# 959AI994/Multi-Gate-VAE

Hardware: AMD Instinct MI355X
Metric: circuit-graphs/sec (train step), AIG-64k batch=64 per GPU (higher is better)
Workload: dtype f32 storage; dense products as bf16x3 split-precision MFMA, fp32 accumulate; 1 GPU; cfg2: DG_AE --type aig, 64 x 65536-node synthetic levelised DAGs per GPU (N=4194304, E=6558720, 120 levels), H=64, 4+4 rounds, layernorm, weights [1,4,4], negatives sampled; step includes the 7-scalar metrics copy (pinned, read one step behind); global_batch=64, parallelism=dp1

## Files before the change

include/mgvae_hip.h:

```cpp
#ifndef MGVAE_HIP_H
#define MGVAE_HIP_H
#include <stdint.h>
#ifdef __cplusplus
extern "C" {
#endif

#ifndef MGV_OK
#define MGV_OK 0
#define MGV_EINVAL (-1)
#define MGV_EUNSUPPORTED (-2)
#endif

int mgv_abi_version(void);

int mgv_struct_stage_fwd(int H, int64_t N, const float* h_in, const int32_t* nbr_ptr, const int32_t* nbr_idx,
                         const uint8_t* xcls, const float* xtab, int C, const float* Wc, const float* bc,
                         const float* Whh, const float* bhh, const float* ln_w, const float* ln_b, float ln_eps,
                         float* h_out, void* stream);
int mgv_struct_stage_bwd(int H, int64_t N, const float* h_in, const int32_t* nbr_ptr, const int32_t* nbr_idx,
                         const uint8_t* xcls, const float* xtab, int C, const float* Wc, const float* WcT,
                         const float* bc, const float* Whh, const float* WhhT, const float* bhh,
                         const float* ln_w, const float* ln_b, float ln_eps, const float* gy_direct,
                         const float* gy_agg, float* g_direct_out, float* g_agg_out, float* dWc, float* dbc,
                         float* dWhh, float* dbhh, float* dxtab, float* dln_w, float* dln_b, void* stream);
// ... 100 lines not shown
                          int skip_inactive_longer_than ,
                          int heavy_active_n, const int32_t* heavy_nodes, const int32_t* heavy_node_seg_ptr, const int32_t* heavy_seg_e0,
                          const int32_t* heavy_seg_e1, const int32_t* heavy_lvl_k_ptr_host, const int32_t* heavy_lvl_seg_ptr_host,
                          float* heavy_ws, int skip_active_longer_than,
                          const float* gh, const float* h_prev, float* d_gh, float* g_hprev, void* stream);

int mgv_attn_pool_fwd(int W, int64_t N, const int32_t* in_ptr, const int32_t* in_src, const float* x, const float* u,
                      float* zbar, float* mstat, float* inv, void* stream);
int mgv_attn_pool_bwd(int W, int64_t N, const int32_t* in_ptr, const int32_t* in_src, const float* x, const float* u,
                      const float* zbar, const float* mstat, const float* inv, const float* dzbar, float* dx, float* du,
                      void* stream);

int mgv_sweep_pull_heavy(int H, int K, const int32_t* nodes, const int32_t* node_seg_ptr, int S, const int32_t* seg_e0,
                         const int32_t* seg_e1, const int32_t* out_dst, const int32_t* out_slot, const uint8_t* gslot,
                         const float* alpha, const float* dsc, const float* dzb, const float* attn_u, float* partial_ws,
                         float* ghs, void* stream);

int mgv_edge_dot_fwd(int H, int64_t E, const float* s, const float* t, int ld, const int64_t* src,
                     const int64_t* dst, int sigmoid, float* out, void* stream);
int mgv_edge_dot_bwd(int H, int64_t E, const float* s, const float* t, int ld, const int64_t* src,
                     const int64_t* dst, int sigmoid, const float* gout, float* ds, float* dt, void* stream);
int mgv_pair_scores_fwd(int H, int64_t M, int64_t N, const float* s, int lds, const float* t, int ldt, int sigmoid, float* out,
                        int64_t ldo, void* stream);
int mgv_pair_scores_bwd(int H, int64_t M, int64_t N, const float* s, int lds, const float* t, int ldt, int sigmoid, const float* out,
                        int64_t ldo, const float* gout, int64_t ldg, float* ds, int ldds, float* dt, int lddt, void* stream);
int mgv_pair_scores_at(int H, int64_t E, const float* s, int lds, const float* t, int ldt, const int64_t* src, const int64_t* dst,
                       int sigmoid, float* out, void* stream);
int mgv_pair_topk(int H, int64_t N, const float* s, int lds, const float* t, int ldt, const int32_t* graph_ptr, int G, int k, int sigmoid,
                  float threshold, int skip_self, int32_t* idx, float* score, int32_t* n_above, void* stream);
int mgv_recon_loss_fwd(int H, const float* s, const float* t, int ld, const int64_t* pos_src, const int64_t* pos_dst,
                       int64_t Epos, const int64_t* neg_src, const int64_t* neg_dst, int64_t Eneg,
                       double* sums, uint64_t* counts, int32_t* pred_bin, double* workspace, int64_t workspace_doubles,
                       void* stream);
int mgv_recon_loss_bwd(int H, int64_t N, const float* s, const float* t, int ld, const int64_t* pos_src, const int64_t* pos_dst,
                       int64_t Epos, const int32_t* pos_out_ptr, const int32_t* pos_out_dst, const int32_t* pos_in_ptr,
                       const int32_t* pos_in_src, const int64_t* neg_src, const int64_t* neg_dst, int64_t Eneg,
                       const float* gscale, float* ds, float* dt, void* stream);
int mgv_recon_loss_bwd_csr(int H, int64_t N, const float* s, const float* t, int ld, const int32_t* pos_out_ptr,
                           const int32_t* pos_out_dst, const int32_t* pos_in_ptr, const int32_t* pos_in_src, int64_t Epos,
                           const int32_t* neg_out_ptr, const int32_t* neg_out_dst, const int32_t* neg_in_ptr,
                           const int32_t* neg_in_src, int64_t Eneg, const float* gscale, float* ds, float* dt,
                           int skip_pos_longer_than , void* stream);
int mgv_recon_heavy_lists(int H, const float* s, const float* t, int ld, int64_t Epos, const float* gscale, int K,
                          const int32_t* nodes, const int32_t* node_seg_ptr, int S, const int32_t* seg_node, const int32_t* seg_e0,
                          const int32_t* seg_e1, const int32_t* list, int which, float* partial_ws, float* out, void* stream);
int mgv_link_keys(int H, const float* s, const float* t, int ld, const int64_t* pos_src, const int64_t* pos_dst, int64_t P,
                  const int64_t* neg_src, const int64_t* neg_dst, int64_t Q, uint32_t* keys, float* scores, int32_t* status,
                  void* stream);
int mgv_link_rank_work_ints(int64_t n);
int mgv_link_rank(int64_t n, int64_t P, const uint32_t* sorted_keys, const int32_t* order, double* out, int32_t* work,
                  int64_t work_ints, void* stream);
int mgv_neg_sample(int64_t N, int64_t E, uint64_t seed, const int32_t* pos_out_ptr, const int32_t* pos_out_dst,
                   int64_t* neg_src, int64_t* neg_dst, int32_t* cnt_out, int32_t* cnt_in, int32_t* rank_out, int32_t* rank_in,
                   void* stream);
int mgv_neg_bucket(int64_t E, const int64_t* neg_src, const int64_t* neg_dst, const int32_t* out_ptr, const int32_t* in_ptr,
                   const int32_t* rank_out, const int32_t* rank_in, int64_t* srt_src, int64_t* srt_dst, int32_t* out_dst, int32_t* in_src,
                   void* stream);

int mgv_func_loss_fwd(int H, int64_t P, const float* hf, const int64_t* pair_a, const int64_t* pair_b,
                      const float* tt, float eps, float* dis, double* ws, double* workspace, int64_t workspace_doubles,
                      void* stream);
int mgv_func_loss_bwd_csr(int H, int64_t N, int64_t P, const float* hf, const int64_t* pair_a, const int64_t* pair_b, const float* tt_sim,
                          const float* dis, float eps, const double* workspace8, const float* grad_loss, const int32_t* a_ptr,
                          const int32_t* a_pair, const int32_t* b_ptr, const int32_t* b_pair, const float* add, float* dhf, void* stream);
int mgv_func_loss_bwd(int H, int64_t P, const float* hf, const int64_t* pair_a, const int64_t* pair_b,
                      const float* tt, const float* dis, float eps, const double* ws, const float* gscale,
                      float* dhf, void* stream);

int mgv_reparam_fwd(int64_t n, const float* mu, const float* logstd, const float* eps, uint64_t seed,
                    float* eps_out, float* z, double* klsum, void* stream);
int mgv_reparam_bwd(int64_t n, const float* mu, const float* logstd, const float* eps, const float* gz,
                    const float* gkl, float klcoef, float* dmu, float* dlogstd, void* stream);
int mgv_confusion(int64_t n, const int32_t* pred_bin, const int32_t* gt_bin, uint64_t* counts, void* stream);

int mgv_sum_workspace_doubles(void);
int mgv_colstats(int64_t N, int C, const float* Y, int ld, double* sums, double* workspace, int64_t workspace_doubles, void* stream);
int mgv_bn_act_fwd(int64_t N, int C, const float* Y, const float* mean, const float* invstd, const float* gamma,
                   const float* beta, float p_drop, uint64_t seed, float* A, void* stream);
int mgv_bn_act_bwd(int64_t N, int C, const float* Y, const float* mean, const float* invstd, const float* gamma,
                   const float* beta, float p_drop, uint64_t seed, const float* dA, float* dZ, double* sums, double* workspace,
                   int64_t workspace_doubles, void* stream);
int mgv_bn_bwd_apply(int64_t N, int C, const float* Y, const float* mean, const float* invstd, const float* gamma,
                     const float* dZ, const double* sums, int batch_stats, float* dY, void* stream);
int mgv_readout_head_fwd(int64_t N, int C, const float* A, const float* w, const float* b, int clamp01, float* prob, void* stream);
int mgv_readout_head_bwd(int64_t N, int C, const float* A, const float* w, const float* b, int clamp01, const float* dprob,
                         float* dA, float* dw, float* db, double* workspace, int64_t workspace_doubles, void* stream);
int mgv_readout_fused_pack_elems(void);
int mgv_readout_fused_grad_floats(void);
int mgv_readout_fused_ws_doubles(int64_t N);
int mgv_readout_fused_fwd(int64_t N, const float* hf, const void* wpack, const float* b1, const float* g1, const float* be1,
// ... 75 lines not shown
```

multi-gate-vae_amd/csrc/losses.hip:

```cpp
#include "mgv_common.h"
#include "mgv_slab.h"
#include "../../include/mgvae_hip.h"

namespace mgv {

__device__ __forceinline__ void atomic_add4(float* p, const float4& v) {
    atomicAdd(p + 0, v.x); atomicAdd(p + 1, v.y); atomicAdd(p + 2, v.z); atomicAdd(p + 3, v.w);
}

__device__ __forceinline__ double block_sum_d(double v, double* red) {
    const int tid = threadIdx.x;
    __syncthreads();
    red[tid] = v;
    __syncthreads();
    for (int s = kThreads / 2; s > 0; s >>= 1) {
        if (tid < s) red[tid] += red[tid + s];
        __syncthreads();
    }
    return red[0];
}

template <int H, bool BWD>
__global__ __launch_bounds__(kThreads) void k_edge_dot(int64_t E, const float* s, const float* t, int ld,
                                                       const int64_t* src, const int64_t* dst, int sigmoid,
// ... 179 lines not shown
        }
        st4(ds + u * ld + 4 * lr, gs);
        st4(dt + u * ld + 4 * lr, gt);
    }
}

template <int H>
__global__ __launch_bounds__(256) void k_recon_heavy_seg(int S, const int32_t* seg_node, const int32_t* seg_e0, const int32_t* seg_e1,
                                                         const int32_t* nodes, const float* s, const float* t, int ld, const int32_t* list,
                                                         int which, int64_t Ep, const float* gscale, float* partial) {
    constexpr int LPR = H / 4, G = 256 / LPR;
    __shared__ __attribute__((aligned(16))) float s_p[G][H];
    const int lr = threadIdx.x % LPR, grp = threadIdx.x / LPR;
    const float wp = -(*gscale) / (float)Ep;
    for (int sg = blockIdx.x; sg < S; sg += gridDim.x) {
        const int64_t u = nodes[seg_node[sg]];
        const float4 own = ld4((which ? t : s) + u * ld + 4 * lr);
        const float* other = which ? s : t;
        float4 acc = zero4();
        for (int e = seg_e0[sg] + grp; e < seg_e1[sg]; e += G) {
            const float4 v = ld4(other + (int64_t)list[e] * ld + 4 * lr);
            const float p = sigmoidf_(group_sum<LPR>(dot4(own, v)));
            acc = fma4(wp * p * (1.0f - p) / (p + 1e-15f), v, acc);
        }
        __syncthreads();
        st4(&s_p[grp][4 * lr], acc);
        __syncthreads();
        if (grp == 0) {
            float4 tot = zero4();
            for (int g = 0; g < G; ++g) tot = add4(tot, ld4(&s_p[g][4 * lr]));
            st4(partial + (int64_t)sg * H + 4 * lr, tot);
        }
    }
}

template <int H>
__global__ __launch_bounds__(kThreads) void k_recon_bwd_rows(int64_t E, const float* s, const float* t, int ld, const int64_t* src,
                                                             const int64_t* dst, int negative, float wscale, const float* gscale,
                                                             float* ds, float* dt) {
    constexpr int EPB = kThreads / H;
    const int l = threadIdx.x % H, slot = threadIdx.x / H;
    const float w = (*gscale) * wscale;
    for (int64_t e0 = (int64_t)blockIdx.x * EPB; e0 < E; e0 += (int64_t)gridDim.x * EPB) {
        const int64_t e = e0 + slot;
        const bool ok = e < E;
        int64_t u = 0, v = 0;
        float x = 0.f, y = 0.f;
        if (ok) { u = src[e]; v = dst[e]; x = s[u * ld + l]; y = t[v * ld + l]; }
        const float p = sigmoidf_(group_sum<H>(x * y));
        if (!ok) continue;
        const float dp = p * (1.0f - p);
        const float c = negative ? w * dp / ((1.0f - p) + 1e-15f) : -w * dp / (p + 1e-15f);
        atomicAdd(ds + u * ld + l, c * y);
        atomicAdd(dt + v * ld + l, c * x);
    }
}

template <int H>
__global__ __launch_bounds__(kThreads) void k_func_dist(int64_t P, const float* hf, const int64_t* pa, const int64_t* pb,
                                                        const float* tt, float eps, float* dis, double* slab) {
    constexpr int LPR = H / 4, PPB = kThreads / LPR;
    __shared__ double red[kThreads];
    const int lr = threadIdx.x % LPR, slot = threadIdx.x / LPR;
    double sd = 0, sd2 = 0, st = 0, st2 = 0;
    for (int64_t p0 = (int64_t)blockIdx.x * PPB; p0 < P; p0 += (int64_t)gridDim.x * PPB) {
        const int64_t p = p0 + slot;
// ... 194 lines not shown
}

extern "C" int mgv_edge_dot_bwd(int H, int64_t E, const float* s, const float* t, int ld, const int64_t* src,
                                const int64_t* dst, int sigmoid, const float* gout, float* ds, float* dt, void* stream) {
    MGV_CHECK_ARG(E >= 0 && s && t && gout && ds && dt && ld >= H && ld % 4 == 0);
    if (E == 0) return MGV_OK;
    MGV_CHECK_ARG(src && dst);
    hipStream_t st = static_cast<hipStream_t>(stream);
    MGV_DISPATCH_H(H, hipLaunchKernelGGL((mgv::k_edge_dot<HH, true>), dim3(mgv::items_grid(E, mgv::kThreads / (HH / 4))), dim3(mgv::kThreads), 0, st,
                                         E, s, t, ld, src, dst, sigmoid, nullptr, gout, ds, dt));
    MGV_LAUNCH_RET();
}

extern "C" int mgv_recon_loss_fwd(int H, const float* s, const float* t, int ld, const int64_t* pos_src, const int64_t* pos_dst,
                                  int64_t Epos, const int64_t* neg_src, const int64_t* neg_dst, int64_t Eneg,
                                  double* sums, uint64_t* counts, int32_t* pred_bin, double* workspace, int64_t workspace_doubles,
                                  void* stream) {
    MGV_CHECK_ARG(s && t && sums && counts && Epos >= 0 && Eneg >= 0 && ld >= H && ld % 4 == 0);
    MGV_CHECK_ARG((Epos == 0 || (pos_src && pos_dst)) && (Eneg == 0 || (neg_src && neg_dst)));
    if (Epos + Eneg == 0) return MGV_OK;
    mgv::ReconArgs a{};
    a.s = s; a.t = t; a.ld = ld; a.psrc = pos_src; a.pdst = pos_dst; a.Ep = Epos; a.nsrc = neg_src; a.ndst = neg_dst; a.En = Eneg;
    a.sums = sums; a.cnt = reinterpret_cast<unsigned long long*>(counts); a.pred_bin = pred_bin;
    hipStream_t st = static_cast<hipStream_t>(stream);
    int grid = 0;
    MGV_DISPATCH_H(H, grid = mgv::items_grid(Epos + Eneg, mgv::kThreads / (HH / 4)));
    MGV_CHECK_ARG(workspace && workspace_doubles >= 2 * (int64_t)grid);
    a.slab = workspace;
    MGV_DISPATCH_H(H, hipLaunchKernelGGL((mgv::k_recon<HH, false>), dim3(grid), dim3(mgv::kThreads), 0, st, a));
    mgv::launch_slab_sum<double, double>(workspace, grid, 2, 2, sums, st);
    MGV_LAUNCH_RET();
}

extern "C" int mgv_recon_loss_bwd(int H, int64_t N, const float* s, const float* t, int ld, const int64_t* pos_src, const int64_t* pos_dst,
                                  int64_t Epos, const int32_t* pos_out_ptr, const int32_t* pos_out_dst, const int32_t* pos_in_ptr,
                                  const int32_t* pos_in_src, const int64_t* neg_src, const int64_t* neg_dst, int64_t Eneg,
                                  const float* gscale, float* ds, float* dt, void* stream) {
    MGV_CHECK_ARG(s && t && gscale && ds && dt && Epos >= 0 && Eneg >= 0 && N >= 0 && ld >= H && ld % 4 == 0);
    MGV_CHECK_ARG((Epos == 0 || (pos_src && pos_dst)) && (Eneg == 0 || (neg_src && neg_dst)));
    const bool pull = pos_out_ptr != nullptr;
    MGV_CHECK_ARG(!pull || (pos_in_ptr && (Epos == 0 || (pos_out_dst && pos_in_src))));
    if (H != 16 && H != 32 && H != 64) return MGV_EUNSUPPORTED;
    hipStream_t st = static_cast<hipStream_t>(stream);
    if (Epos > 0 && pull) {
        MGV_DISPATCH_H(H, hipLaunchKernelGGL((mgv::k_recon_bwd_pull<HH>), dim3(mgv::items_grid(N, mgv::kThreads / (HH / 4))), dim3(mgv::kThreads), 0, st,
                                             N, s, t, ld, pos_out_ptr, pos_out_dst, pos_in_ptr, pos_in_src, Epos, gscale, ds, dt));
    }
    for (int neg = (Epos > 0 && pull) ? 1 : 0; neg < 2; ++neg) {
        const int64_t E = neg ? Eneg : Epos;
        if (E == 0) continue;
        const int64_t* es = neg ? neg_src : pos_src;
        const int64_t* ed = neg ? neg_dst : pos_dst;
        const float wsc = 1.0f / (float)E;
        switch (H) {
            case 16: hipLaunchKernelGGL((mgv::k_recon_bwd_rows<16>), dim3(mgv::items_grid(E, mgv::kThreads / 16)), dim3(mgv::kThreads), 0, st, E, s, t, ld, es, ed, neg, wsc, gscale, ds, dt); break;
            case 32: hipLaunchKernelGGL((mgv::k_recon_bwd_rows<32>), dim3(mgv::items_grid(E, mgv::kThreads / 32)), dim3(mgv::kThreads), 0, st, E, s, t, ld, es, ed, neg, wsc, gscale, ds, dt); break;
            case 64: hipLaunchKernelGGL((mgv::k_recon_bwd_rows<64>), dim3(mgv::items_grid(E, mgv::kThreads / 64)), dim3(mgv::kThreads), 0, st, E, s, t, ld, es, ed, neg, wsc, gscale, ds, dt); break;
            default: return MGV_EUNSUPPORTED;
        }
    }
    MGV_LAUNCH_RET();
}

extern "C" int mgv_recon_loss_bwd_csr(int H, int64_t N, const float* s, const float* t, int ld, const int32_t* pos_out_ptr,
                                      const int32_t* pos_out_dst, const int32_t* pos_in_ptr, const int32_t* pos_in_src, int64_t Epos,
                                      const int32_t* neg_out_ptr, const int32_t* neg_out_dst, const int32_t* neg_in_ptr,
// ... 98 lines not shown
```

multi-gate-vae_amd/csrc/neg_sample.hip:

```cpp
#include "mgv_common.h"
#include "../../include/mgvae_hip.h"

namespace mgv {

__device__ __forceinline__ uint64_t splitmix64(uint64_t x) {
    x += 0x9E3779B97F4A7C15ull;
    x = (x ^ (x >> 30)) * 0xBF58476D1CE4E5B9ull;
    x = (x ^ (x >> 27)) * 0x94D049BB133111EBull;
    return x ^ (x >> 31);
}

__global__ __launch_bounds__(kThreads) void k_neg_sample(int64_t N, int64_t E, uint64_t seed, const int32_t* out_ptr, const int32_t* out_dst,
                                                        int64_t* neg_src, int64_t* neg_dst, int32_t* cnt_out, int32_t* cnt_in,
                                                        int32_t* rank_out, int32_t* rank_in) {
    for (int64_t i = (int64_t)blockIdx.x * kThreads + threadIdx.x; i < E; i += (int64_t)gridDim.x * kThreads) {
        uint64_t ctr = seed ^ ((uint64_t)i * 0xD1342543DE82EF95ull);
        int s, d;
        for (int attempt = 0;; ++attempt) {
            const uint64_t r = splitmix64(ctr + attempt);
            s = (int)(((r >> 32) * (uint64_t)N) >> 32);
            d = (int)(((r & 0xFFFFFFFFull) * (uint64_t)N) >> 32);
            bool ok = s != d;
            if (ok)
                for (int e = out_ptr[s]; e < out_ptr[s + 1]; ++e)
                    if (out_dst[e] == d) { ok = false; break; }
            if (ok || attempt >= 64) break;
        }
        neg_src[i] = s; neg_dst[i] = d;
        rank_out[i] = atomicAdd(cnt_out + s, 1);
        rank_in[i] = atomicAdd(cnt_in + d, 1);
    }
}

__global__ __launch_bounds__(kThreads) void k_neg_bucket(int64_t E, const int64_t* neg_src, const int64_t* neg_dst, const int32_t* out_ptr,
                                                        const int32_t* in_ptr, const int32_t* rank_out, const int32_t* rank_in, int64_t* srt_src,
                                                        int64_t* srt_dst, int32_t* out_dst, int32_t* in_src) {
    for (int64_t i = (int64_t)blockIdx.x * kThreads + threadIdx.x; i < E; i += (int64_t)gridDim.x * kThreads) {
        const int s = (int)neg_src[i], d = (int)neg_dst[i];
        const int p = out_ptr[s] + rank_out[i];
        srt_src[p] = s; srt_dst[p] = d; out_dst[p] = d;
        in_src[in_ptr[d] + rank_in[i]] = s;
    }
}

}

extern "C" int mgv_neg_sample(int64_t N, int64_t E, uint64_t seed, const int32_t* pos_out_ptr, const int32_t* pos_out_dst,
                              int64_t* neg_src, int64_t* neg_dst, int32_t* cnt_out, int32_t* cnt_in, int32_t* rank_out, int32_t* rank_in,
                              void* stream) {
    MGV_CHECK_ARG(N >= 2 && N < (1ll << 31) && E >= 0 && pos_out_ptr && neg_src && neg_dst && cnt_out && cnt_in && rank_out && rank_in);
    if (E == 0) return MGV_OK;
    hipLaunchKernelGGL(mgv::k_neg_sample, dim3(mgv::grid_for((E + mgv::kThreads - 1) / mgv::kThreads, 16)), dim3(mgv::kThreads), 0,
                       static_cast<hipStream_t>(stream), N, E, seed, pos_out_ptr, pos_out_dst, neg_src, neg_dst, cnt_out, cnt_in, rank_out, rank_in);
    MGV_LAUNCH_RET();
}

extern "C" int mgv_neg_bucket(int64_t E, const int64_t* neg_src, const int64_t* neg_dst, const int32_t* out_ptr, const int32_t* in_ptr,
                              const int32_t* rank_out, const int32_t* rank_in, int64_t* srt_src, int64_t* srt_dst, int32_t* out_dst, int32_t* in_src,
                              void* stream) {
    MGV_CHECK_ARG(E >= 0 && out_ptr && in_ptr && rank_out && rank_in);
    if (E == 0) return MGV_OK;
    MGV_CHECK_ARG(neg_src && neg_dst && srt_src && srt_dst && out_dst && in_src);
    hipLaunchKernelGGL(mgv::k_neg_bucket, dim3(mgv::grid_for((E + mgv::kThreads - 1) / mgv::kThreads, 16)), dim3(mgv::kThreads), 0,
                       static_cast<hipStream_t>(stream), E, neg_src, neg_dst, out_ptr, in_ptr, rank_out, rank_in, srt_src, srt_dst, out_dst, in_src);
    MGV_LAUNCH_RET();
}
```

multi-gate-vae_amd/deepgate/_model_base.py:

```python
import os

import torch
from torch import nn

from . import ops
from .arch.mlp import MLP
from .arch.tfmlp import TFMlpAggr
from .data import plan_of
from .digae_layer import DirectedInnerProductDecoder
from .sampling import NegativeEdges, negative_sampling, negative_sampling_device

EPS = 1e-15
DEVICE_SAMPLER = True
MAX_LOGSTD = 10


class FunctionalModel(nn.Module):
    ENCODER_ATTR = 'struct_encoder'
    GATES = ()

    def __init__(self, struct_encoder, num_rounds=1, dim_hidden=128, enable_encode=True, enable_reverse=True):
        super().__init__()
        setattr(self, self.ENCODER_ATTR, struct_encoder)
        self.decoder = DirectedInnerProductDecoder()
# ... 73 lines not shown
    def _decoder_halves(self, hs):
        st = ops.linear(hs.detach(), self.hs_decompose.weight, self.hs_decompose.bias)
        H = st.shape[1] // 2
        return st[:, :H], st[:, H:]

    def predict_links(self, hs, k, graph_ptr=None, skip_self=True):
        with torch.no_grad():
            s, t = self._decoder_halves(hs)
            return ops.pair_topk(s, t, k, graph_ptr=graph_ptr, sigmoid=True, threshold=0.5, skip_self=skip_self)

    def reconstruction_counts(self, hs, edge_index, graph_ptr, threshold=0.5):
        with torch.no_grad():
            s, t = self._decoder_halves(hs)
            return ops.reconstruction_counts(s, t, edge_index, graph_ptr, threshold)

    def recon_loss(self, hs, pos_edge_index, neg_edge_index=None, want_pred=True, edge_keys=None, plan=None, pass_hs=False, want_rank=False):
        if pass_hs and hs.requires_grad:
            st, self._hs_pass = ops.linear_passthrough(hs, self.hs_decompose.weight, self.hs_decompose.bias)
        else:
            st = ops.linear(hs, self.hs_decompose.weight, self.hs_decompose.bias)
        if plan is not None and (plan.E != pos_edge_index.shape[1] or plan.N != hs.shape[0]):
            plan = None
        neg_csr = None
        if neg_edge_index is None:
            neg_edge_index = self._draw_negatives(hs, pos_edge_index, plan, edge_keys)
        if plan is not None and hs.is_cuda and torch.is_tensor(neg_edge_index) and neg_edge_index.shape[1] > 0:
            cache = getattr(plan, '_neg_cache', None)
            key = (neg_edge_index.data_ptr(), neg_edge_index._version, tuple(neg_edge_index.shape), hs.shape[0])
            if cache is None or cache[0] is not neg_edge_index or cache[1] != key:
                from .sampling import bucket_negatives
                cache = plan._neg_cache = (neg_edge_index, key, bucket_negatives(neg_edge_index.long(), hs.shape[0]))
            neg_edge_index = cache[2]
        if isinstance(neg_edge_index, NegativeEdges):
            neg_csr, neg_edge_index = neg_edge_index.csr, neg_edge_index.edge_index
        loss, counts, pred_bin = ops.ReconLossFn.apply(st, pos_edge_index, neg_edge_index, want_pred, plan, neg_csr)
        self.last_confusion = counts
        self.last_link_metrics = ops.link_record(st, None, pos_edge_index, neg_edge_index) if want_rank else None
        Ep, En = pos_edge_index.shape[1], neg_edge_index.shape[1]
        gt_bin = None
        if want_pred:
            gt_bin = torch.zeros(Ep + En, dtype=torch.int32, device=hs.device)
            gt_bin[:Ep] = 1
        return loss, pred_bin if want_pred else None, gt_bin

    def load(self, model_path):
        checkpoint = torch.load(model_path, map_location=lambda storage, loc: storage)
        src = checkpoint['state_dict']
        state = {}
        for k, v in src.items():
            state[k[7:] if k.startswith('module') and not k.startswith('module_list') else k] = v
        own = self.state_dict()
        for k in list(state):
            if k in own:
                if state[k].shape != own[k].shape:
                    print('Skip loading parameter {}, required shape{}, loaded shape{}.'.format(k, own[k].shape, state[k].shape))
                    state[k] = own[k]
            else:
                print('Drop parameter {}.'.format(k))
        for k in own:
            if k not in state:
                print('No param {}.'.format(k))
                state[k] = own[k]
        self.load_state_dict(state, strict=False)

    def load_pretrained(self, pretrained_model_path=''):
        if pretrained_model_path == '':
            pretrained_model_path = os.path.join(os.path.dirname(__file__), 'pretrained', 'model.pth')
        self.load(pretrained_model_path)
```

multi-gate-vae_amd/deepgate/ops.py:

```python
import torch

from . import _hip
from ._hip import HipLibraryError, check, ptr

import os

F32 = torch.float32
I32 = torch.int32
U8 = torch.uint8
LN_EPS = 1e-5

PRECISION = os.environ.get('MGV_PRECISION', 'x3')
FIRST_STAGE_TABLE = True


def use_x3(H):
    return PRECISION == 'x3' and H in (32, 64)


def split_bf16(w):
    hi = w.to(torch.bfloat16)
    lo = (w - hi.to(torch.float32)).to(torch.bfloat16)
    return hi, lo

# ... 913 lines not shown
              ptr(idx), ptr(score), ptr(n_above))
    return idx, score, n_above


def reconstruction_counts(s, t, edge_index, graph_ptr, threshold=0.5):
    dev = s.device
    gp = torch.as_tensor(graph_ptr).to(device=dev, dtype=torch.int64)
    G = gp.numel() - 1
    src, dst = _edge_rows(edge_index)
    _, _, n_above = pair_topk(s, t, 1, graph_ptr=gp, sigmoid=True, threshold=threshold, skip_self=False)
    if G <= 0:
        return torch.zeros((0, 4), dtype=torch.int64, device=dev)
    hit = (pair_scores_at(s, t, edge_index, sigmoid=True) > threshold).to(torch.int64)
    gid = torch.bucketize(src, gp[1:].contiguous(), right=True).clamp_(max=G - 1)
    tp = torch.zeros(G, dtype=torch.int64, device=dev).index_add_(0, gid, hit)
    edges = torch.zeros(G, dtype=torch.int64, device=dev).index_add_(0, gid, torch.ones_like(hit))
    cs = torch.zeros(s.shape[0] + 1, dtype=torch.int64, device=dev)
    cs[1:] = torch.cumsum(n_above.to(torch.int64), 0)
    n = gp[1:] - gp[:-1]
    return torch.stack([tp, cs[gp[1:]] - cs[gp[:-1]], edges, n * n], dim=1)


def dense_scores(s, t):
    return pair_scores(s, t, sigmoid=False)


class ReconLossFn(torch.autograd.Function):

    @staticmethod
    def forward(ctx, st, pos_edge_index, neg_edge_index, want_pred, plan=None, neg_csr=None):
        std = check(st.detach().contiguous(), F32, 'st')
        N, H2 = std.shape
        H = H2 // 2
        ps, pd = _edge_rows(pos_edge_index)
        ns, nd = _edge_rows(neg_edge_index)
        Ep, En = ps.numel(), ns.numel()
        dev = std.device
        sums = torch.zeros(2, dtype=torch.float64, device=dev)
        counts = torch.zeros(4, dtype=torch.int64, device=dev)
        pred = torch.empty(Ep + En, dtype=torch.int32, device=dev) if want_pred else None
        t_view = std[:, H:]
        _hip.call('mgv_recon_loss_fwd', H, ptr(std), ptr(t_view), H2, ptr(ps), ptr(pd), Ep, ptr(ns), ptr(nd), En,
                  ptr(sums), ptr(counts), ptr(pred), *_sw(std.device))
        loss = (sums[0] / max(Ep, 1) + sums[1] / max(En, 1)).to(F32)
        ctx.save_for_backward(std, ps, pd, ns, nd)
        ctx.plan, ctx.neg_csr = plan, neg_csr
        ctx.mark_non_differentiable(counts)
        if pred is not None:
            ctx.mark_non_differentiable(pred)
            return loss, counts, pred
        return loss, counts, torch.empty(0, dtype=torch.int32, device=dev)

    @staticmethod
    def backward(ctx, gloss, _gc, _gp):
        global _SWEEP_BWD_EVENT
        if _SWEEP_BWD_EVENT is not None and gloss.is_cuda:
            torch.cuda.current_stream().wait_event(_SWEEP_BWD_EVENT)
            _SWEEP_BWD_EVENT = None
        std, ps, pd, ns, nd = ctx.saved_tensors
        H2 = std.shape[1]
        H = H2 // 2
        g = gloss.detach().to(F32).reshape(1).contiguous()
        pl = ctx.plan
        if pl is not None and ctx.neg_csr is not None:
            dst_ = torch.empty_like(std)
            heavy = [(0, pl.heavy_segments(True), pl.out_dst), (1, pl.heavy_segments(False), pl.in_src)]
            skip = pl.HEAVY_ROW if any(hv is not None for _, hv, _ in heavy) else 0
            _hip.call('mgv_recon_loss_bwd_csr', H, std.shape[0], ptr(std), ptr(std[:, H:]), H2, ptr(pl.out_ptr), ptr(pl.out_dst),
                      ptr(pl.in_ptr), ptr(pl.in_src), ps.numel(), *[ptr(c) for c in ctx.neg_csr], ns.numel(), ptr(g), ptr(dst_),
                      ptr(dst_[:, H:]), skip)
            for which, hv, lst in heavy:
                if hv is not None:
                    pw = workspace(hv['S'] * H, std.device)
                    _hip.call('mgv_recon_heavy_lists', H, ptr(std), ptr(std[:, H:]), H2, ps.numel(), ptr(g), hv['K'], ptr(hv['nodes']),
                              ptr(hv['node_seg_ptr']), hv['S'], ptr(hv['seg_node']), ptr(hv['seg_e0']), ptr(hv['seg_e1']), ptr(lst), which,
                              ptr(pw), ptr(dst_[:, H:]) if which else ptr(dst_))
            return dst_, None, None, None, None, None
        dst_ = torch.zeros_like(std)
        csr = (pl.out_ptr, pl.out_dst, pl.in_ptr, pl.in_src) if pl is not None else (None, None, None, None)
        _hip.call('mgv_recon_loss_bwd', H, std.shape[0], ptr(std), ptr(std[:, H:]), H2, ptr(ps), ptr(pd), ps.numel(),
                  *[ptr(c) for c in csr], ptr(ns), ptr(nd), ns.numel(), ptr(g), ptr(dst_), ptr(dst_[:, H:]))
        return dst_, None, None, None, None, None


def confusion_counts(pred_bin, gt_bin):
    counts = torch.zeros(4, dtype=torch.int64, device=pred_bin.device)
    _hip.call('mgv_confusion', pred_bin.numel(), ptr(check(pred_bin.contiguous(), torch.int32, 'pred_bin')),
              ptr(check(gt_bin.contiguous(), torch.int32, 'gt_bin')), ptr(counts))
    return counts


LINK_RECORD_WORDS = 8


def link_record(st_or_s, t=None, pos_edge_index=None, neg_edge_index=None, return_scores=False):
    neg = getattr(neg_edge_index, 'edge_index', neg_edge_index)
    P, Q = int(pos_edge_index.shape[1]), int(neg.shape[1])
    if P == 0 or Q == 0:
        raise ValueError('Only one class present (%d positive, %d negative pairs): ROC-AUC and average precision are not defined' % (P, Q))
    sd = check(st_or_s.detach().contiguous(), F32, 'st' if t is None else 's')
    if t is None:
        ld = sd.shape[1]
        H = ld // 2
        td = sd[:, H:]
    else:
        td = check(t.detach().contiguous(), F32, 't')
        ld = H = sd.shape[1]
        if td.shape != sd.shape:
            raise HipLibraryError('s and t must have the same shape (got %s and %s)' % (tuple(sd.shape), tuple(td.shape)))
    n = P + Q
# ... 288 lines not shown
```

multi-gate-vae_amd/deepgate/sampling.py:

```python
import itertools

import torch

from . import _hip
from ._hip import ptr

_CALLS = itertools.count()


class NegativeEdges:

    def __init__(self, edge_index, out_ptr, out_dst, in_ptr, in_src):
        self.edge_index, self.out_ptr, self.out_dst, self.in_ptr, self.in_src = edge_index, out_ptr, out_dst, in_ptr, in_src

    @property
    def csr(self):
        return self.out_ptr, self.out_dst, self.in_ptr, self.in_src


def bucket_negatives(neg, N):
    dev = neg.device
    E = int(neg.shape[1])
    i32 = dict(dtype=torch.int32, device=dev)
    src, dst = neg[0].contiguous(), neg[1].contiguous()
    in_ptr, out_ptr = torch.empty(N + 1, **i32), torch.empty(N + 1, **i32)
    in_src, in_dst, out_dst, out_slot = (torch.empty(max(E, 1), **i32) for _ in range(4))
    n_s = _hip.call_value('mgv_plan_csr_scratch_ints', N, E)
    scratch = torch.empty(n_s, **i32)
    status = torch.empty(2, **i32)
    _hip.call('mgv_plan_csr', N, E, ptr(src), ptr(dst), ptr(in_ptr), ptr(in_src), ptr(in_dst), ptr(out_ptr), ptr(out_dst), ptr(out_slot),
              None, None, ptr(scratch), n_s, ptr(status))
    if int(status[0].item()) != 0:
        raise ValueError('neg_edge_index holds node ids outside [0, num_nodes)')
    counts = (out_ptr[1:] - out_ptr[:-1]).long()
    srt_src = torch.repeat_interleave(torch.arange(N, device=dev), counts, output_size=E)
    srt = torch.stack([srt_src, out_dst[:E].long()])
    return NegativeEdges(srt, out_ptr, out_dst, in_ptr, in_src)


def negative_sampling_device(plan, num_neg_samples=None, generator=None):
    N, dev = plan.N, plan.device
    if getattr(plan, 'num_self_loops', None) is None:
        plan.count_self_loops()
    E = (plan.E - plan.num_self_loops) + N if num_neg_samples is None else int(num_neg_samples)
    base = generator.initial_seed() if generator is not None else torch.initial_seed()
    seed = (base * 0x9E3779B97F4A7C15 + next(_CALLS) * 0xD1B54A32D192ED03 + 0x2545F4914F6CDD1D) & 0xFFFFFFFFFFFFFFFF
    scratch = torch.zeros(2, N, dtype=torch.int32, device=dev)
    neg = torch.empty(2, E, dtype=torch.int64, device=dev)
    rank = torch.empty(2, max(E, 1), dtype=torch.int32, device=dev)
    _hip.call('mgv_neg_sample', N, E, seed, ptr(plan.out_ptr), ptr(plan.out_dst), ptr(neg[0]), ptr(neg[1]), ptr(scratch[0]), ptr(scratch[1]),
              ptr(rank[0]), ptr(rank[1]))
    ptrs = torch.zeros(2, N + 1, dtype=torch.int32, device=dev)
    for k in range(2):
        ptrs[k, 1:] = torch.cumsum(scratch[k], 0, dtype=torch.int32)
    srt = torch.empty(2, E, dtype=torch.int64, device=dev)
    out_dst = torch.empty(max(E, 1), dtype=torch.int32, device=dev)
    in_src = torch.empty(max(E, 1), dtype=torch.int32, device=dev)
    _hip.call('mgv_neg_bucket', E, ptr(neg[0]), ptr(neg[1]), ptr(ptrs[0]), ptr(ptrs[1]), ptr(rank[0]), ptr(rank[1]),
              ptr(srt[0]), ptr(srt[1]), ptr(out_dst), ptr(in_src))
    ss = torch.empty(N + 1 + E, dtype=torch.int32, device=dev)
    _hip.call('mgv_sort_lists_i32', N, E, ptr(ptrs[0]), ptr(out_dst), ptr(ss), ss.numel())
    _hip.call('mgv_sort_lists_i32', N, E, ptr(ptrs[1]), ptr(in_src), ptr(ss), ss.numel())
    srt[1].copy_(out_dst[:E])
    return NegativeEdges(srt, ptrs[0], out_dst, ptrs[1], in_src)


def sorted_edge_keys(pos_edge_index, num_nodes):
    src, dst = pos_edge_index[0].long(), pos_edge_index[1].long()
    keep = src != dst
    return torch.sort(src[keep] * int(num_nodes) + dst[keep]).values


def negative_sampling(pos_edge_index, num_nodes, num_neg_samples=None, generator=None, keys=None):
    dev = pos_edge_index.device
    N = int(num_nodes)
    if keys is None:
        keys = sorted_edge_keys(pos_edge_index, N)
    want = int(keys.numel()) + N if num_neg_samples is None else int(num_neg_samples)
    out = torch.empty((2, 0), dtype=torch.long, device=dev)
    guard = 0
    while out.shape[1] < want:
        m = want - out.shape[1]
        m = m + m // 8 + 16
        s = torch.randint(0, N, (m,), device=dev, generator=generator)
        d = torch.randint(0, N, (m,), device=dev, generator=generator)
        k = s * N + d
        ok = s != d
        if keys.numel() > 0:
            pos = torch.searchsorted(keys, k).clamp_(max=keys.numel() - 1)
            ok &= keys[pos] != k
        out = torch.cat([out, torch.stack([s[ok], d[ok]])], dim=1)
        guard += 1
        if guard > 64:
            raise RuntimeError('negative_sampling: graph too dense to draw %d non-edges' % want)
    return out[:, :want].contiguous()
```

Before: 982.3 graphs/s.

## Compute recon loss forward from CSR lists and sample negatives as packed int32

```diff
diff --git a/include/mgvae_hip.h b/include/mgvae_hip.h
--- a/include/mgvae_hip.h
+++ b/include/mgvae_hip.h
@@ -156,6 +156,11 @@
                        int64_t Epos, const int64_t* neg_src, const int64_t* neg_dst, int64_t Eneg,
                        double* sums, uint64_t* counts, int32_t* pred_bin, double* workspace, int64_t workspace_doubles,
                        void* stream);
+int mgv_recon_loss_fwd_csr(int H, int64_t N, const float* s, const float* t, int ld, const int32_t* pos_out_ptr,
+                           const int32_t* pos_out_dst, int64_t Epos, const int32_t* neg_out_ptr, const int32_t* neg_out_dst,
+                           int64_t Eneg, int skip_pos_longer_than, const int32_t* heavy_nodes, int S, const int32_t* seg_node,
+                           const int32_t* seg_e0, const int32_t* seg_e1, double* sums, uint64_t* counts, double* workspace,
+                           int64_t workspace_doubles, void* stream);
 int mgv_recon_loss_bwd(int H, int64_t N, const float* s, const float* t, int ld, const int64_t* pos_src, const int64_t* pos_dst,
                        int64_t Epos, const int32_t* pos_out_ptr, const int32_t* pos_out_dst, const int32_t* pos_in_ptr,
                        const int32_t* pos_in_src, const int64_t* neg_src, const int64_t* neg_dst, int64_t Eneg,
@@ -180,6 +185,10 @@
 int mgv_neg_bucket(int64_t E, const int64_t* neg_src, const int64_t* neg_dst, const int32_t* out_ptr, const int32_t* in_ptr,
                    const int32_t* rank_out, const int32_t* rank_in, int64_t* srt_src, int64_t* srt_dst, int32_t* out_dst, int32_t* in_src,
                    void* stream);
+int mgv_neg_sample_i32(int64_t N, int64_t E, uint64_t seed, const int32_t* pos_out_ptr, const int32_t* pos_out_dst,
+                       int32_t* pair, int32_t* cnt_out, int32_t* cnt_in, int32_t* rank, void* stream);
+int mgv_neg_bucket_i32(int64_t E, const int32_t* pair, const int32_t* out_ptr, const int32_t* in_ptr, const int32_t* rank,
+                       int32_t* out_dst, int32_t* in_src, void* stream);
 
 int mgv_func_loss_fwd(int H, int64_t P, const float* hf, const int64_t* pair_a, const int64_t* pair_b,
                       const float* tt, float eps, float* dis, double* ws, double* workspace, int64_t workspace_doubles,
diff --git a/multi-gate-vae_amd/csrc/losses.hip b/multi-gate-vae_amd/csrc/losses.hip
--- a/multi-gate-vae_amd/csrc/losses.hip
+++ b/multi-gate-vae_amd/csrc/losses.hip
@@ -235,6 +235,111 @@
             st4(partial + (int64_t)sg * H + 4 * lr, tot);
         }
     }
+}
+
+__device__ __forceinline__ float dot4_pairwise_rounded(const float4& a, const float4& b) {
+#pragma clang fp contract(off)
+    const float p0 = a.x * b.x, p1 = a.y * b.y, p2 = a.z * b.z, p3 = a.w * b.w;
+    return ((p0 + p1) + p2) + p3;
+}
+
+struct ReconTally {
+    double lp = 0, ln = 0;
+    unsigned int tp = 0, fp = 0, tn = 0, fn = 0;
+    __device__ __forceinline__ void add(float p, bool pos) {
+        const bool hit = p > 0.5f;
+        if (pos) { lp += (double)(-logf(p + 1e-15f)); tp += hit; fn += !hit; }
+        else     { ln += (double)(-logf((1.0f - p) + 1e-15f)); fp += hit; tn += !hit; }
+    }
+    __device__ __forceinline__ void flush(double* red, double* row, unsigned long long* cnt) {
+        const double sp = block_sum_d(lp, red), sn = block_sum_d(ln, red);
+        const double c0 = block_sum_d((double)tp, red), c1 = block_sum_d((double)fp, red);
+        const double c2 = block_sum_d((double)tn, red), c3 = block_sum_d((double)fn, red);
+        if (threadIdx.x == 0) {
+            row[0] = sp; row[1] = sn;
+            if (c0 > 0) atomicAdd(cnt + 0, (unsigned long long)c0);
+            if (c1 > 0) atomicAdd(cnt + 1, (unsigned long long)c1);
+            if (c2 > 0) atomicAdd(cnt + 2, (unsigned long long)c2);
+            if (c3 > 0) atomicAdd(cnt + 3, (unsigned long long)c3);
+        }
+    }
+};
+
+template <int H>
+__global__ __launch_bounds__(kThreads) void k_recon_fwd_lists(int64_t N, const float* s, const float* t, int ld, const int32_t* pout_ptr,
+                                                              const int32_t* pout_dst, int64_t Ep, const int32_t* nout_ptr,
+                                                              const int32_t* nout_dst, int64_t En, int skip_len, double* slab,
+                                                              unsigned long long* cnt) {
+    constexpr int LPR = H / 4, RPB = kThreads / LPR, K = 4;
+    __shared__ double red[kThreads];
+    const int lr = threadIdx.x % LPR, slot = threadIdx.x / LPR;
+    int64_t first, end, stride;
+    if ((gridDim.x & 7) == 0) {
+        const int64_t chunk = ((N + 8 * RPB - 1) / (8 * RPB)) * RPB;
+        first = (blockIdx.x & 7) * chunk + (int64_t)(blockIdx.x >> 3) * RPB;
+        end = min(N, ((blockIdx.x & 7) + 1) * chunk);
+        stride = (int64_t)(gridDim.x >> 3) * RPB;
+    } else {
+        first = (int64_t)blockIdx.x * RPB; end = N; stride = (int64_t)gridDim.x * RPB;
+    }
+    ReconTally tally;
+    for (int64_t n0 = first; n0 < end; n0 += stride) {
+        const int64_t u = n0 + slot;
+        if (u >= end) continue;
+        int b0 = 0, b1 = 0, c0 = 0, c1 = 0;
+        if (Ep > 0) {
+            b0 = pout_ptr[u]; c0 = pout_ptr[u + 1] - b0;
+            if (skip_len > 0 && c0 > skip_len) c0 = 0;
+        }
+        if (En > 0) { b1 = nout_ptr[u]; c1 = nout_ptr[u + 1] - b1; }
+        c1 += c0;
+        if (c1 == 0) continue;
+        const float4 su = ld4(s + u * ld + 4 * lr);
+        auto partner = [&](int j) -> int { return j < c0 ? pout_dst[b0 + j] : nout_dst[b1 + (j - c0)]; };
+        int id[K];
+#pragma unroll
+        for (int k = 0; k < K; ++k) id[k] = k < c1 ? partner(k) : 0;
+        for (int j0 = 0; j0 < c1; j0 += K) {
+            float4 v[K];
+#pragma unroll
+            for (int k = 0; k < K; ++k)
+                if (j0 + k < c1) v[k] = ld4(t + (int64_t)id[k] * ld + 4 * lr);
+            int nid[K];
+#pragma unroll
+            for (int k = 0; k < K; ++k) nid[k] = j0 + K + k < c1 ? partner(j0 + K + k) : 0;
+#pragma unroll
+            for (int k = 0; k < K; ++k) {
+                const int j = j0 + k;
+                if (j < c1) {
+                    const float p = sigmoidf_(group_sum<LPR>(dot4_pairwise_rounded(su, v[k])));
+                    if (lr == 0) tally.add(p, j < c0);
+                }
+            }
+#pragma unroll
+            for (int k = 0; k < K; ++k) id[k] = nid[k];
+        }
+    }
+    tally.flush(red, slab + 2 * (int64_t)blockIdx.x, cnt);
+}
+
+template <int H>
+__global__ __launch_bounds__(kThreads) void k_recon_fwd_heavy_seg(int S, const int32_t* seg_node, const int32_t* seg_e0, const int32_t* seg_e1,
+                                                                  const int32_t* nodes, const float* s, const float* t, int ld,
+                                                                  const int32_t* list, double* slab, unsigned long long* cnt) {
+    constexpr int LPR = H / 4, G = kThreads / LPR;
+    __shared__ double red[kThreads];
+    const int lr = threadIdx.x % LPR, grp = threadIdx.x / LPR;
+    ReconTally tally;
+    for (int sg = blockIdx.x; sg < S; sg += gridDim.x) {
+        const int64_t u = nodes[seg_node[sg]];
+        const float4 su = ld4(s + u * ld + 4 * lr);
+        for (int e = seg_e0[sg] + grp; e < seg_e1[sg]; e += G) {
+            const float4 v = ld4(t + (int64_t)list[e] * ld + 4 * lr);
+            const float p = sigmoidf_(group_sum<LPR>(dot4_pairwise_rounded(su, v)));
+            if (lr == 0) tally.add(p, true);
+        }
+    }
+    tally.flush(red, slab + 2 * (int64_t)blockIdx.x, cnt);
 }
 
 template <int H>
@@ -495,6 +600,31 @@
     MGV_LAUNCH_RET();
 }
 
+extern "C" int mgv_recon_loss_fwd_csr(int H, int64_t N, const float* s, const float* t, int ld, const int32_t* pos_out_ptr,
+                                      const int32_t* pos_out_dst, int64_t Epos, const int32_t* neg_out_ptr, const int32_t* neg_out_dst,
+                                      int64_t Eneg, int skip_pos_longer_than, const int32_t* heavy_nodes, int S, const int32_t* seg_node,
+                                      const int32_t* seg_e0, const int32_t* seg_e1, double* sums, uint64_t* counts, double* workspace,
+                                      int64_t workspace_doubles, void* stream) {
+    MGV_CHECK_ARG(s && t && sums && counts && Epos >= 0 && Eneg >= 0 && N >= 0 && ld >= H && ld % 4 == 0 && skip_pos_longer_than >= 0 && S >= 0);
+    MGV_CHECK_ARG(Epos == 0 || (pos_out_ptr && pos_out_dst));
+    MGV_CHECK_ARG(Eneg == 0 || (neg_out_ptr && neg_out_dst));
+    MGV_CHECK_ARG((skip_pos_longer_than > 0) == (S > 0) && (S == 0 || (Epos > 0 && heavy_nodes && seg_node && seg_e0 && seg_e1)));
+    if (H != 16 && H != 32 && H != 64 && H != 128) return MGV_EUNSUPPORTED;
+    if (N == 0 || Epos + Eneg == 0) return MGV_OK;
+    const int grid = mgv::items_grid(N, mgv::kThreads / (H / 4)), hgrid = S < 2048 ? S : 2048;
+    MGV_CHECK_ARG(workspace && workspace_doubles >= 2 * (int64_t)(grid + hgrid));
+    hipStream_t st = static_cast<hipStream_t>(stream);
+    unsigned long long* cnt = reinterpret_cast<unsigned long long*>(counts);
+    MGV_DISPATCH_H(H, hipLaunchKernelGGL((mgv::k_recon_fwd_lists<HH>), dim3(grid), dim3(mgv::kThreads), 0, st, N, s, t, ld, pos_out_ptr, pos_out_dst,
+                                         Epos, neg_out_ptr, neg_out_dst, Eneg, skip_pos_longer_than, workspace, cnt));
+    if (S > 0) {
+        MGV_DISPATCH_H(H, hipLaunchKernelGGL((mgv::k_recon_fwd_heavy_seg<HH>), dim3(hgrid), dim3(mgv::kThreads), 0, st, S, seg_node, seg_e0, seg_e1,
+                                             heavy_nodes, s, t, ld, pos_out_dst, workspace + 2 * (int64_t)grid, cnt));
+    }
+    mgv::launch_slab_sum<double, double>(workspace, grid + hgrid, 2, 2, sums, st);
+    MGV_LAUNCH_RET();
+}
+
 extern "C" int mgv_recon_loss_bwd(int H, int64_t N, const float* s, const float* t, int ld, const int64_t* pos_src, const int64_t* pos_dst,
                                   int64_t Epos, const int32_t* pos_out_ptr, const int32_t* pos_out_dst, const int32_t* pos_in_ptr,
                                   const int32_t* pos_in_src, const int64_t* neg_src, const int64_t* neg_dst, int64_t Eneg,
diff --git a/multi-gate-vae_amd/csrc/neg_sample.hip b/multi-gate-vae_amd/csrc/neg_sample.hip
--- a/multi-gate-vae_amd/csrc/neg_sample.hip
+++ b/multi-gate-vae_amd/csrc/neg_sample.hip
@@ -43,6 +43,59 @@
     }
 }
 
+__global__ __launch_bounds__(kThreads) void k_neg_sample_i32(int64_t N, int64_t E, uint64_t seed, const int32_t* out_ptr, const int32_t* out_dst,
+                                                            int2* pair, int32_t* cnt_out, int32_t* cnt_in, int2* rank) {
+    for (int64_t i = (int64_t)blockIdx.x * kThreads + threadIdx.x; i < E; i += (int64_t)gridDim.x * kThreads) {
+        uint64_t ctr = seed ^ ((uint64_t)i * 0xD1342543DE82EF95ull);
+        int s, d;
+        for (int attempt = 0;; ++attempt) {
+            const uint64_t r = splitmix64(ctr + attempt);
+            s = (int)(((r >> 32) * (uint64_t)N) >> 32);
+            d = (int)(((r & 0xFFFFFFFFull) * (uint64_t)N) >> 32);
+            bool ok = s != d;
+            if (ok)
+                for (int e = out_ptr[s]; e < out_ptr[s + 1]; ++e)
+                    if (out_dst[e] == d) { ok = false; break; }
+            if (ok || attempt >= 64) break;
+        }
+        pair[i] = make_int2(s, d);
+        const int ro = atomicAdd(cnt_out + s, 1), ri = atomicAdd(cnt_in + d, 1);
+        rank[i] = make_int2(ro, ri);
+    }
+}
+
+__global__ __launch_bounds__(kThreads) void k_neg_bucket_i32(int64_t E, const int2* pair, const int32_t* out_ptr, const int32_t* in_ptr,
+                                                            const int2* rank, int32_t* out_dst, int32_t* in_src) {
+    for (int64_t i = (int64_t)blockIdx.x * kThreads + threadIdx.x; i < E; i += (int64_t)gridDim.x * kThreads) {
+        const int2 p = pair[i], r = rank[i];
+        out_dst[out_ptr[p.x] + r.x] = p.y;
+        in_src[in_ptr[p.y] + r.y] = p.x;
+    }
+}
+
+}
+
+extern "C" int mgv_neg_sample_i32(int64_t N, int64_t E, uint64_t seed, const int32_t* pos_out_ptr, const int32_t* pos_out_dst,
+                                  int32_t* pair, int32_t* cnt_out, int32_t* cnt_in, int32_t* rank, void* stream) {
+    MGV_CHECK_ARG(N >= 2 && N < (1ll << 31) && E >= 0 && E < (1ll << 31) && pos_out_ptr && pair && cnt_out && cnt_in && rank);
+    MGV_CHECK_ARG((reinterpret_cast<uintptr_t>(pair) & 7) == 0 && (reinterpret_cast<uintptr_t>(rank) & 7) == 0);
+    if (E == 0) return MGV_OK;
+    hipLaunchKernelGGL(mgv::k_neg_sample_i32, dim3(mgv::grid_for((E + mgv::kThreads - 1) / mgv::kThreads, 16)), dim3(mgv::kThreads), 0,
+                       static_cast<hipStream_t>(stream), N, E, seed, pos_out_ptr, pos_out_dst, reinterpret_cast<int2*>(pair), cnt_out, cnt_in,
+                       reinterpret_cast<int2*>(rank));
+    MGV_LAUNCH_RET();
+}
+
+extern "C" int mgv_neg_bucket_i32(int64_t E, const int32_t* pair, const int32_t* out_ptr, const int32_t* in_ptr, const int32_t* rank,
+                                  int32_t* out_dst, int32_t* in_src, void* stream) {
+    MGV_CHECK_ARG(E >= 0 && E < (1ll << 31) && out_ptr && in_ptr);
+    if (E == 0) return MGV_OK;
+    MGV_CHECK_ARG(pair && rank && out_dst && in_src);
+    MGV_CHECK_ARG((reinterpret_cast<uintptr_t>(pair) & 7) == 0 && (reinterpret_cast<uintptr_t>(rank) & 7) == 0);
+    hipLaunchKernelGGL(mgv::k_neg_bucket_i32, dim3(mgv::grid_for((E + mgv::kThreads - 1) / mgv::kThreads, 16)), dim3(mgv::kThreads), 0,
+                       static_cast<hipStream_t>(stream), E, reinterpret_cast<const int2*>(pair), out_ptr, in_ptr,
+                       reinterpret_cast<const int2*>(rank), out_dst, in_src);
+    MGV_LAUNCH_RET();
 }
 
 extern "C" int mgv_neg_sample(int64_t N, int64_t E, uint64_t seed, const int32_t* pos_out_ptr, const int32_t* pos_out_dst,
diff --git a/multi-gate-vae_amd/deepgate/_model_base.py b/multi-gate-vae_amd/deepgate/_model_base.py
--- a/multi-gate-vae_amd/deepgate/_model_base.py
+++ b/multi-gate-vae_amd/deepgate/_model_base.py
@@ -129,11 +129,13 @@
                 cache = plan._neg_cache = (neg_edge_index, key, bucket_negatives(neg_edge_index.long(), hs.shape[0]))
             neg_edge_index = cache[2]
         if isinstance(neg_edge_index, NegativeEdges):
-            neg_csr, neg_edge_index = neg_edge_index.csr, neg_edge_index.edge_index
+            neg_csr, En = neg_edge_index.csr, neg_edge_index.num_edges
+        else:
+            En = neg_edge_index.shape[1]
         loss, counts, pred_bin = ops.ReconLossFn.apply(st, pos_edge_index, neg_edge_index, want_pred, plan, neg_csr)
         self.last_confusion = counts
         self.last_link_metrics = ops.link_record(st, None, pos_edge_index, neg_edge_index) if want_rank else None
-        Ep, En = pos_edge_index.shape[1], neg_edge_index.shape[1]
+        Ep = pos_edge_index.shape[1]
         gt_bin = None
         if want_pred:
             gt_bin = torch.zeros(Ep + En, dtype=torch.int32, device=hs.device)
diff --git a/multi-gate-vae_amd/deepgate/ops.py b/multi-gate-vae_amd/deepgate/ops.py
--- a/multi-gate-vae_amd/deepgate/ops.py
+++ b/multi-gate-vae_amd/deepgate/ops.py
@@ -969,19 +969,31 @@
         std = check(st.detach().contiguous(), F32, 'st')
         N, H2 = std.shape
         H = H2 // 2
-        ps, pd = _edge_rows(pos_edge_index)
-        ns, nd = _edge_rows(neg_edge_index)
-        Ep, En = ps.numel(), ns.numel()
         dev = std.device
         sums = torch.zeros(2, dtype=torch.float64, device=dev)
         counts = torch.zeros(4, dtype=torch.int64, device=dev)
-        pred = torch.empty(Ep + En, dtype=torch.int32, device=dev) if want_pred else None
         t_view = std[:, H:]
-        _hip.call('mgv_recon_loss_fwd', H, ptr(std), ptr(t_view), H2, ptr(ps), ptr(pd), Ep, ptr(ns), ptr(nd), En,
-                  ptr(sums), ptr(counts), ptr(pred), *_sw(std.device))
+        ctx.plan, ctx.neg_csr = plan, neg_csr
+        neg_pairs = getattr(neg_edge_index, 'num_edges', None)
+        if plan is not None and neg_csr is not None and not want_pred:
+            Ep, En = int(pos_edge_index.shape[1]), neg_pairs if neg_pairs is not None else int(neg_edge_index.shape[1])
+            hv = plan.heavy_segments(True)
+            heavy = (plan.HEAVY_ROW, ptr(hv['nodes']), hv['S'], ptr(hv['seg_node']), ptr(hv['seg_e0']), ptr(hv['seg_e1'])) if hv is not None \
+                else (0, None, 0, None, None, None)
+            _hip.call('mgv_recon_loss_fwd_csr', H, N, ptr(std), ptr(t_view), H2, ptr(plan.out_ptr), ptr(plan.out_dst), Ep, ptr(neg_csr[0]),
+                      ptr(neg_csr[1]), En, *heavy, ptr(sums), ptr(counts), *_sw(dev))
+            pred = None
+            ctx.save_for_backward(std)
+        else:
+            ps, pd = _edge_rows(pos_edge_index)
+            ns, nd = _edge_rows(neg_edge_index.edge_index if neg_pairs is not None else neg_edge_index)
+            Ep, En = ps.numel(), ns.numel()
+            pred = torch.empty(Ep + En, dtype=torch.int32, device=dev) if want_pred else None
+            _hip.call('mgv_recon_loss_fwd', H, ptr(std), ptr(t_view), H2, ptr(ps), ptr(pd), Ep, ptr(ns), ptr(nd), En,
+                      ptr(sums), ptr(counts), ptr(pred), *_sw(dev))
+            ctx.save_for_backward(std, ps, pd, ns, nd)
+        ctx.n_pairs = (Ep, En)
         loss = (sums[0] / max(Ep, 1) + sums[1] / max(En, 1)).to(F32)
-        ctx.save_for_backward(std, ps, pd, ns, nd)
-        ctx.plan, ctx.neg_csr = plan, neg_csr
         ctx.mark_non_differentiable(counts)
         if pred is not None:
             ctx.mark_non_differentiable(pred)
@@ -994,7 +1006,8 @@
         if _SWEEP_BWD_EVENT is not None and gloss.is_cuda:
             torch.cuda.current_stream().wait_event(_SWEEP_BWD_EVENT)
             _SWEEP_BWD_EVENT = None
-        std, ps, pd, ns, nd = ctx.saved_tensors
+        std, *pairs = ctx.saved_tensors
+        Ep, En = ctx.n_pairs
         H2 = std.shape[1]
         H = H2 // 2
         g = gloss.detach().to(F32).reshape(1).contiguous()
@@ -1004,15 +1017,16 @@
             heavy = [(0, pl.heavy_segments(True), pl.out_dst), (1, pl.heavy_segments(False), pl.in_src)]
             skip = pl.HEAVY_ROW if any(hv is not None for _, hv, _ in heavy) else 0
             _hip.call('mgv_recon_loss_bwd_csr', H, std.shape[0], ptr(std), ptr(std[:, H:]), H2, ptr(pl.out_ptr), ptr(pl.out_dst),
-                      ptr(pl.in_ptr), ptr(pl.in_src), ps.numel(), *[ptr(c) for c in ctx.neg_csr], ns.numel(), ptr(g), ptr(dst_),
+                      ptr(pl.in_ptr), ptr(pl.in_src), Ep, *[ptr(c) for c in ctx.neg_csr], En, ptr(g), ptr(dst_),
                       ptr(dst_[:, H:]), skip)
             for which, hv, lst in heavy:
                 if hv is not None:
                     pw = workspace(hv['S'] * H, std.device)
-                    _hip.call('mgv_recon_heavy_lists', H, ptr(std), ptr(std[:, H:]), H2, ps.numel(), ptr(g), hv['K'], ptr(hv['nodes']),
+                    _hip.call('mgv_recon_heavy_lists', H, ptr(std), ptr(std[:, H:]), H2, Ep, ptr(g), hv['K'], ptr(hv['nodes']),
                               ptr(hv['node_seg_ptr']), hv['S'], ptr(hv['seg_node']), ptr(hv['seg_e0']), ptr(hv['seg_e1']), ptr(lst), which,
                               ptr(pw), ptr(dst_[:, H:]) if which else ptr(dst_))
             return dst_, None, None, None, None, None
+        ps, pd, ns, nd = pairs
         dst_ = torch.zeros_like(std)
         csr = (pl.out_ptr, pl.out_dst, pl.in_ptr, pl.in_src) if pl is not None else (None, None, None, None)
         _hip.call('mgv_recon_loss_bwd', H, std.shape[0], ptr(std), ptr(std[:, H:]), H2, ptr(ps), ptr(pd), ps.numel(),
diff --git a/multi-gate-vae_amd/deepgate/sampling.py b/multi-gate-vae_amd/deepgate/sampling.py
--- a/multi-gate-vae_amd/deepgate/sampling.py
+++ b/multi-gate-vae_amd/deepgate/sampling.py
@@ -10,12 +10,26 @@
 
 class NegativeEdges:
 
-    def __init__(self, edge_index, out_ptr, out_dst, in_ptr, in_src):
-        self.edge_index, self.out_ptr, self.out_dst, self.in_ptr, self.in_src = edge_index, out_ptr, out_dst, in_ptr, in_src
+    def __init__(self, edge_index, out_ptr, out_dst, in_ptr, in_src, num_edges=None):
+        self._edge_index, self.out_ptr, self.out_dst, self.in_ptr, self.in_src = edge_index, out_ptr, out_dst, in_ptr, in_src
+        self.num_edges = int(edge_index.shape[1]) if edge_index is not None else int(num_edges)
 
     @property
     def csr(self):
         return self.out_ptr, self.out_dst, self.in_ptr, self.in_src
+
+    @property
+    def edge_index(self):
+        if self._edge_index is None:
+            self._edge_index = pairs_by_source(self.out_ptr, self.out_dst, self.num_edges)
+        return self._edge_index
+
+
+def pairs_by_source(out_ptr, out_dst, E):
+    N = out_ptr.numel() - 1
+    counts = (out_ptr[1:] - out_ptr[:-1]).long()
+    src = torch.repeat_interleave(torch.arange(N, device=out_ptr.device), counts, output_size=E)
+    return torch.stack([src, out_dst[:E].long()])
 
 
 def bucket_negatives(neg, N):
@@ -32,10 +46,7 @@
               None, None, ptr(scratch), n_s, ptr(status))
     if int(status[0].item()) != 0:
         raise ValueError('neg_edge_index holds node ids outside [0, num_nodes)')
-    counts = (out_ptr[1:] - out_ptr[:-1]).long()
-    srt_src = torch.repeat_interleave(torch.arange(N, device=dev), counts, output_size=E)
-    srt = torch.stack([srt_src, out_dst[:E].long()])
-    return NegativeEdges(srt, out_ptr, out_dst, in_ptr, in_src)
+    return NegativeEdges(pairs_by_source(out_ptr, out_dst, E), out_ptr, out_dst, in_ptr, in_src)
 
 
 def negative_sampling_device(plan, num_neg_samples=None, generator=None):
@@ -45,24 +56,21 @@
     E = (plan.E - plan.num_self_loops) + N if num_neg_samples is None else int(num_neg_samples)
     base = generator.initial_seed() if generator is not None else torch.initial_seed()
     seed = (base * 0x9E3779B97F4A7C15 + next(_CALLS) * 0xD1B54A32D192ED03 + 0x2545F4914F6CDD1D) & 0xFFFFFFFFFFFFFFFF
-    scratch = torch.zeros(2, N, dtype=torch.int32, device=dev)
-    neg = torch.empty(2, E, dtype=torch.int64, device=dev)
-    rank = torch.empty(2, max(E, 1), dtype=torch.int32, device=dev)
-    _hip.call('mgv_neg_sample', N, E, seed, ptr(plan.out_ptr), ptr(plan.out_dst), ptr(neg[0]), ptr(neg[1]), ptr(scratch[0]), ptr(scratch[1]),
-              ptr(rank[0]), ptr(rank[1]))
-    ptrs = torch.zeros(2, N + 1, dtype=torch.int32, device=dev)
+    i32 = dict(dtype=torch.int32, device=dev)
+    counts = torch.zeros(2, N, **i32)
+    pair = torch.empty(max(E, 1), 2, **i32)
+    rank = torch.empty(max(E, 1), 2, **i32)
+    _hip.call('mgv_neg_sample_i32', N, E, seed, ptr(plan.out_ptr), ptr(plan.out_dst), ptr(pair), ptr(counts[0]), ptr(counts[1]), ptr(rank))
+    ptrs = torch.empty(2, N + 1, **i32)
+    ss = torch.empty(N + 1 + E, **i32)
     for k in range(2):
-        ptrs[k, 1:] = torch.cumsum(scratch[k], 0, dtype=torch.int32)
-    srt = torch.empty(2, E, dtype=torch.int64, device=dev)
-    out_dst = torch.empty(max(E, 1), dtype=torch.int32, device=dev)
-    in_src = torch.empty(max(E, 1), dtype=torch.int32, device=dev)
-    _hip.call('mgv_neg_bucket', E, ptr(neg[0]), ptr(neg[1]), ptr(ptrs[0]), ptr(ptrs[1]), ptr(rank[0]), ptr(rank[1]),
-              ptr(srt[0]), ptr(srt[1]), ptr(out_dst), ptr(in_src))
-    ss = torch.empty(N + 1 + E, dtype=torch.int32, device=dev)
+        _hip.call('mgv_scan_exclusive_i32', N, ptr(counts[k]), ptr(ptrs[k]), ptr(ss))
+    out_dst = torch.empty(max(E, 1), **i32)
+    in_src = torch.empty(max(E, 1), **i32)
+    _hip.call('mgv_neg_bucket_i32', E, ptr(pair), ptr(ptrs[0]), ptr(ptrs[1]), ptr(rank), ptr(out_dst), ptr(in_src))
     _hip.call('mgv_sort_lists_i32', N, E, ptr(ptrs[0]), ptr(out_dst), ptr(ss), ss.numel())
     _hip.call('mgv_sort_lists_i32', N, E, ptr(ptrs[1]), ptr(in_src), ptr(ss), ss.numel())
-    srt[1].copy_(out_dst[:E])
-    return NegativeEdges(srt, ptrs[0], out_dst, ptrs[1], in_src)
+    return NegativeEdges(None, ptrs[0], out_dst, ptrs[1], in_src, num_edges=E)
 
 
 def sorted_edge_keys(pos_edge_index, num_nodes):
```

New measurement: 989.3 graphs/s (median of 6 runs). About the same (+0.7%).
